# apchenstu/mvsnerf

Hardware: NVIDIA B200
Metric: rays/sec @ 128 samples, DTU 512x640 (higher is better)
Workload: dtype fp16 operands / fp32 accumulate

## Files before the change

### mvsnerf_b200/csrc/render_tc2.cu

```cuda
#include "render_frontend.cuh"
#include "umma.cuh"

namespace mvsn {

using namespace umma;

namespace tc2 {
constexpr int W_MOD = 0;
constexpr int W_L0 = 8192;
constexpr int W_L1 = 16384;
constexpr int L_STRIDE = 18432;
constexpr int W_L5 = W_L1 + 4 * L_STRIDE;
constexpr int W_V = W_L5 + 3 * 8192;
constexpr int W_V_TILE = 10240;
constexpr int W_RGB = W_V + 12288;
constexpr int HALF_BYTES = W_RGB + 1024;
constexpr int TAIL_OFFSET = 2 * HALF_BYTES;
constexpr int TOTAL_BYTES = TAIL_OFFSET + 16;
static_assert(W_L5 % 1024 == 0 && W_V % 1024 == 0 && W_RGB % 1024 == 0 && HALF_BYTES % 1024 == 0, "SW128 blocks need 1024-byte alignment");
constexpr int N_VIEWS_OP = 80;
}

namespace {

constexpr int THREADS = 544;
constexpr int OFF_SLOT = tc2::HALF_BYTES;
constexpr int SLOT_BYTES = 32768, OFF_PE = 0, OFF_MISC = 16384;
constexpr int OFF_XCH = OFF_SLOT + 2 * SLOT_BYTES;
constexpr int SMEM_BYTES = OFF_XCH + 2 * 2048 + 1024;
constexpr uint32_t COL_H = 128, COL_MOD = 192, COL_LZ = 128;

struct Shared {
    uint64_t in_ready[2];
    uint64_t pe_ready[2];
    uint64_t acc_ready[2];
    uint64_t pe_free[2];
    uint64_t misc_free[2];
    uint64_t w_full;
    uint32_t tmem_base;
    Cams cams;
};

__device__ __forceinline__ uint32_t pack_h2(float a, float b) {
    __half2 h = __floats2half2_rn(a, b);
    return *reinterpret_cast<uint32_t*>(&h);
}
__device__ __forceinline__ void named_bar_sync(int id, int nthreads) {
    asm volatile("bar.sync %0, %1;\n" ::"r"(id), "r"(nthreads) : "memory");
}
__device__ __forceinline__ void tmem_wait16(uint32_t (&r)[16]) {
    asm volatile("tcgen05.wait::ld.sync.aligned;\n"
                 : "+r"(r[0]), "+r"(r[1]), "+r"(r[2]), "+r"(r[3]), "+r"(r[4]), "+r"(r[5]), "+r"(r[6]), "+r"(r[7]),
                   "+r"(r[8]), "+r"(r[9]), "+r"(r[10]), "+r"(r[11]), "+r"(r[12]), "+r"(r[13]), "+r"(r[14]), "+r"(r[15])
                 :: "memory");
}
__device__ __forceinline__ void tmem_wait8(uint32_t (&r)[8]) {
    asm volatile("tcgen05.wait::ld.sync.aligned;\n"
                 : "+r"(r[0]), "+r"(r[1]), "+r"(r[2]), "+r"(r[3]), "+r"(r[4]), "+r"(r[5]), "+r"(r[6]), "+r"(r[7]) :: "memory");
}
__device__ __forceinline__ void tmem_ld8(uint32_t taddr, uint32_t (&r)[8]) {
    asm volatile("tcgen05.ld.sync.aligned.32x32b.x8.b32 {%0, %1, %2, %3, %4, %5, %6, %7}, [%8];\n"
                 : "=r"(r[0]), "=r"(r[1]), "=r"(r[2]), "=r"(r[3]), "=r"(r[4]), "=r"(r[5]), "=r"(r[6]), "=r"(r[7]) : "r"(taddr));
}
__device__ __forceinline__ void tmem_st8(uint32_t taddr, const uint32_t (&r)[8]) {
    asm volatile("tcgen05.st.sync.aligned.32x32b.x8.b32 [%0], {%1, %2, %3, %4, %5, %6, %7, %8};\n"
                 :: "r"(taddr), "r"(r[0]), "r"(r[1]), "r"(r[2]), "r"(r[3]), "r"(r[4]), "r"(r[5]), "r"(r[6]), "r"(r[7]) : "memory");
}

template <bool RELU>
__device__ __forceinline__ uint32_t cvt_h2(float lo, float hi) {
    uint32_t r;
    if (RELU) asm("cvt.rn.relu.satfinite.f16x2.f32 %0, %1, %2;\n" : "=r"(r) : "f"(hi), "f"(lo));
    else      asm("cvt.rn.satfinite.f16x2.f32 %0, %1, %2;\n" : "=r"(r) : "f"(hi), "f"(lo));
    return r;
}
__device__ __forceinline__ uint32_t mul_relu_h2(uint32_t a, uint32_t b) {
    uint32_t r;
    const uint32_t zero = 0u, maxh = 0x7BFF7BFFu;
    asm("fma.rn.relu.f16x2 %0, %1, %2, %3;\n" : "=r"(r) : "r"(a), "r"(b), "r"(zero));
    asm("min.f16x2 %0, %1, %2;\n" : "=r"(r) : "r"(r), "r"(maxh));
    return r;
}

__device__ __forceinline__ void epilogue_hidden(uint32_t t_acc, uint32_t t_mod, uint32_t t_h) {
    uint32_t a[2][16], m[2][8];
    tmem_ld16(t_acc, a[0]);
    tmem_ld8(t_mod, m[0]);
#pragma unroll
    for (int i = 0; i < 8; ++i) {
        tmem_wait16(a[i & 1]);
        tmem_wait8(m[i & 1]);
        if (i + 1 < 8) {
            tmem_ld16(t_acc + (i + 1) * 16, a[(i + 1) & 1]);
            tmem_ld8(t_mod + (i + 1) * 8, m[(i + 1) & 1]);
        }
        uint32_t o[8];
#pragma unroll
        for (int j = 0; j < 8; ++j)
            o[j] = mul_relu_h2(cvt_h2<false>(__uint_as_float(a[i & 1][2 * j]), __uint_as_float(a[i & 1][2 * j + 1])), m[i & 1][j]);
        tmem_st8(t_h + i * 8, o);
    }
}

#ifdef MVSN_TC_TRACE
#define TC_TRACE(ev) do { if (tr && tr_n < 1023) tr[tr_n++] = (clock64() << 8) | (long long)(ev); } while (0)
#else
#define TC_TRACE(ev) do { } while (0)
#endif

template <bool FAST>
__global__ void __cluster_dims__(2, 1, 1) __launch_bounds__(THREADS, 1)
render_tc2_kernel(const SceneDev sc, const RenderIO io, const uint8_t* __restrict__ wimg) {
    extern __shared__ uint8_t smem_raw[];
    uint8_t* smem = smem_raw + ((1024u - (smem_u32(smem_raw) & 1023u)) & 1023u);
    __shared__ Shared sh;
    const int tid = threadIdx.x, warp = tid >> 5, lane = tid & 31;
    const uint32_t rank = cluster_ctarank();

    load_cams(sc, &sh.cams, tid);
    if (tid == 0) {
        for (int s = 0; s < 2; ++s) {
            mbar_init(&sh.in_ready[s], 8);
            mbar_init(&sh.pe_ready[s], 8);
            mbar_init(&sh.acc_ready[s], 1);
            mbar_init(&sh.pe_free[s], 1);
            mbar_init(&sh.misc_free[s], 1);
        }
        mbar_init(&sh.w_full, 1);
        fence_barrier_init();
    }
    if (warp == 16) { tmem_alloc_pair(&sh.tmem_base, 512); tmem_relinquish_pair(); }
    __syncthreads();
    if (tid == 0) {
        mbar_arrive_expect_tx(&sh.w_full, (uint32_t)tc2::HALF_BYTES);
        const uint8_t* src = wimg + (size_t)rank * tc2::HALF_BYTES;
        for (int i = 0; i < 4; ++i) bulk_load(smem + i * 32000, src + i * 32000, 32000u, &sh.w_full);
    }
    mbar_wait(&sh.w_full, 0);
    tc_fence_before();
    __syncthreads();
    cluster_sync_all();
    tc_fence_after();
    const uint32_t tmem = sh.tmem_base;
#ifdef MVSN_TC_TRACE
    long long* tr = nullptr; int tr_n = 0;
    if (io.trace && blockIdx.x == 0 && lane == 0) {
        if (warp < 16 && (warp & 3) == 0) tr = io.trace + (warp >> 2) * 1024;
        else if (warp == 16) tr = io.trace + 4 * 1024;
    }
#endif

    const int N = io.N, S = io.S;
    const int RT = io.rays_per_tile, SP = 128 / RT;
    const int rt_shift = 31 - __clz(RT);
    const int NT = (S + SP - 1) / SP;
    const int G = (N + RT - 1) / RT;
    const int npairs = (int)gridDim.x >> 1, pair = (int)blockIdx.x >> 1;
    const int n_gpass = (G + npairs * 4 - 1) / (npairs * 4);
    auto group_of = [&](int gp, int s, int r) { return ((gp * npairs + pair) * 2 + s) * 2 + r; };
    auto slot_active = [&](int gp, int s) { return group_of(gp, s, 0) < G; };

    if (warp < 8) {
        const int s = warp >> 2, wq = warp & 3, row = wq * 32 + lane;
        const uint32_t t_acc = tmem + ((uint32_t)(wq * 32) << 16) + (uint32_t)(s * 256);
        const uint32_t t_h = t_acc + COL_H, t_mod = t_acc + COL_MOD, t_lz = t_acc + COL_LZ;
        const uint32_t leader_in_ready = mapa_u32(smem_u32(&sh.in_ready[s]), 0);
        uint32_t par_acc = 0;
        float cT = 1.f, c0 = 0.f, c1 = 0.f, c2 = 0.f, c3 = 0.f, c4 = 0.f;
        const float br0 = __ldg(reinterpret_cast<const float*>(wimg + tc2::TAIL_OFFSET));
        const float br1 = __ldg(reinterpret_cast<const float*>(wimg + tc2::TAIL_OFFSET) + 1);
        const float br2 = __ldg(reinterpret_cast<const float*>(wimg + tc2::TAIL_OFFSET) + 2);
        float4* xch = reinterpret_cast<float4*>(smem + OFF_XCH + s * 2048);

        auto signal = [&]() {
            tc_fence_before();
            __syncwarp();
            if (lane == 0) mbar_arrive_cluster(leader_in_ready);
        };
        signal();

#pragma unroll 1
        for (int gp = 0; gp < n_gpass; ++gp) {
            if (!slot_active(gp, s)) continue;
            const int g = group_of(gp, s, (int)rank);
#pragma unroll 1
            for (int tile = 0; tile < NT; ++tile) {
                mbar_wait(&sh.acc_ready[s], par_acc); par_acc ^= 1;
                TC_TRACE(10);
                tc_fence_after();
                {
                    uint32_t mu[32], t[2][16];
                    tmem_ld16(t_lz + 64, t[0]);
#pragma unroll
                    for (int i = 0; i < 4; ++i) {
                        tmem_wait16(t[i & 1]);
                        tmem_ld16(i + 1 < 4 ? t_lz + 64 + (i + 1) * 16 : t_lz, t[(i + 1) & 1]);
#pragma unroll
                        for (int j = 0; j < 8; ++j)
                            mu[i * 8 + j] = cvt_h2<false>(__uint_as_float(t[i & 1][2 * j]), __uint_as_float(t[i & 1][2 * j + 1]));
                    }
#pragma unroll
                    for (int i = 0; i < 4; ++i) {
                        tmem_wait16(t[i & 1]);
                        if (i + 1 < 4) tmem_ld16(t_lz + (i + 1) * 16, t[(i + 1) & 1]);
                        uint32_t o[8];
#pragma unroll
                        for (int j = 0; j < 8; ++j)
                            o[j] = cvt_h2<false>(__uint_as_float(t[i & 1][2 * j]), __uint_as_float(t[i & 1][2 * j + 1]));
                        tmem_st8(t_mod + i * 8, o);
                    }
#pragma unroll
                    for (int i = 0; i < 4; ++i) {
                        uint32_t o[8];
#pragma unroll
                        for (int j = 0; j < 8; ++j) o[j] = mu[i * 8 + j];
                        tmem_st8(t_mod + 32 + i * 8, o);
                    }
                    tmem_st_wait();
                }
                epilogue_hidden(t_acc, t_mod, t_h);
                tmem_st_wait();
                TC_TRACE(30);
                signal();
#pragma unroll 1
                for (int op = 1; op < 6; ++op) {
                    mbar_wait(&sh.acc_ready[s], par_acc); par_acc ^= 1;
                    TC_TRACE(10 + op);
                    tc_fence_after();
                    epilogue_hidden(t_acc, t_mod, t_h);
                    tmem_st_wait();
                    TC_TRACE(30 + op);
                    signal();
                }
                float sigma;
                {
                    mbar_wait(&sh.acc_ready[s], par_acc); par_acc ^= 1;
                    TC_TRACE(16);
                    tc_fence_after();
                    uint32_t a[2][16];
                    tmem_ld16(t_acc, a[0]);
#pragma unroll
                    for (int i = 0; i < 4; ++i) {
                        tmem_wait16(a[i & 1]);
                        tmem_ld16(t_acc + (i + 1) * 16, a[(i + 1) & 1]);
                        uint32_t o[8];
#pragma unroll
                        for (int j = 0; j < 8; ++j)
                            o[j] = cvt_h2<true>(__uint_as_float(a[i & 1][2 * j]), __uint_as_float(a[i & 1][2 * j + 1]));
                        tmem_st8(t_h + i * 8, o);
                    }
                    tmem_wait16(a[0]);
                    sigma = fmaxf(__uint_as_float(a[0][0]), 0.f);
                    tmem_st_wait();
                    TC_TRACE(36);
                    signal();
                }
                float cr, cg, cb;
                {
                    mbar_wait(&sh.acc_ready[s], par_acc); par_acc ^= 1;
                    TC_TRACE(17);
                    tc_fence_after();
                    uint32_t r16[16];
                    tmem_ld16(t_acc, r16);
                    tmem_wait16(r16);
                    signal();
                    cr = __fdividef(1.f, 1.f + __expf(-(__uint_as_float(r16[0]) + br0)));
                    cg = __fdividef(1.f, 1.f + __expf(-(__uint_as_float(r16[1]) + br1)));
                    cb = __fdividef(1.f, 1.f + __expf(-(__uint_as_float(r16[2]) + br2)));
                }
                xch[row] = make_float4(1.f - __expf(-sigma), cr, cg, cb);
                named_bar_sync(1 + s, 128);
                if (row < RT) {
                    if (tile == 0) { cT = 1.f; c0 = c1 = c2 = c3 = c4 = 0.f; }
                    const int cray = g * RT + row;
                    if (cray < N) {
                        float znear = 0.f, zfar = 0.f;
                        if (FAST) { const float4 r1 = __ldg(reinterpret_cast<const float4*>(io.rays + (size_t)cray * 8) + 1); znear = r1.z; zfar = r1.w; }
                        for (int sub = 0; sub < SP; ++sub) {
                            const int sj = tile * SP + sub;
                            if (sj >= S) break;
                            const float4 v = xch[sub * RT + row];
                            float z;
                            if (FAST) {
                                const float t = __ldg(io.t_steps + sj);
                                if (!io.rg.lindisp) z = __fadd_rn(__fmul_rn(znear, 1.f - t), __fmul_rn(zfar, t));
                                else z = __fdiv_rn(1.f, __fadd_rn(__fmul_rn(__fdiv_rn(1.f, znear), 1.f - t), __fmul_rn(__fdiv_rn(1.f, zfar), t)));
                            } else {
                                z = __ldg(io.z + (size_t)cray * S + sj);
                            }
                            const float wgt = v.x * cT;
                            if (io.alpha) io.alpha[(size_t)cray * S + sj] = v.x;
                            if (io.weights) io.weights[(size_t)cray * S + sj] = wgt;
                            c0 = fmaf(wgt, v.y, c0); c1 = fmaf(wgt, v.z, c1); c2 = fmaf(wgt, v.w, c2);
                            c3 = fmaf(wgt, z, c3); c4 += wgt;
                            cT *= (1.f - v.x) + 1e-10f;
                        }
                        if (tile == NT - 1) {
                            float o0 = c0, o1 = c1, o2 = c2;
                            if (sc.white_bkgd) { const float bg = 1.f - c4; o0 += bg; o1 += bg; o2 += bg; }
                            store_pixel(io, cray, o0, o1, o2, c3);
                        }
                    }
                }
                TC_TRACE(53);
            }
        }
    } else if (warp < 16) {
        const int s = (warp - 8) >> 2, row = ((warp - 8) & 3) * 32 + lane;
        uint8_t* slot = smem + OFF_SLOT + s * SLOT_BYTES;
        const uint32_t leader_pe_ready = mapa_u32(smem_u32(&sh.pe_ready[s]), 0);
        uint32_t tcount = 0;
#pragma unroll 1
        for (int gp = 0; gp < n_gpass; ++gp) {
            if (!slot_active(gp, s)) continue;
            const int g = group_of(gp, s, (int)rank);
#pragma unroll 1
            for (int tile = 0; tile < NT; ++tile, ++tcount) {
                TC_TRACE(1);
                const int r_in = row & (RT - 1), s_idx = tile * SP + (row >> rt_shift);
                const int ray = g * RT + r_in;
                const bool valid = g < G && ray < N && s_idx < S;
                const size_t si = (size_t)ray * S + s_idx;
                float nx = 0.f, ny = 0.f, nz = 0.f;
                float px = 0.f, py = 0.f, pz = 0.f, dx = 0.f, dy = 0.f, dz = 1.f;
                if (valid) {
                    if (FAST) {
                        const float4* rp = reinterpret_cast<const float4*>(io.rays + (size_t)ray * 8);
                        const float4 r0 = __ldg(rp), r1 = __ldg(rp + 1);
                        dx = r0.w; dy = r1.x; dz = r1.y;
                        const float near = r1.z, far = r1.w, t = __ldg(io.t_steps + s_idx);
                        float zv;
                        if (!io.rg.lindisp) zv = __fadd_rn(__fmul_rn(near, 1.f - t), __fmul_rn(far, t));
                        else zv = __fdiv_rn(1.f, __fadd_rn(__fmul_rn(__fdiv_rn(1.f, near), 1.f - t),
                                                           __fmul_rn(__fdiv_rn(1.f, far), t)));
                        px = __fadd_rn(r0.x, __fmul_rn(dx, zv));
                        py = __fadd_rn(r0.y, __fmul_rn(dy, zv));
                        pz = __fadd_rn(r0.z, __fmul_rn(dz, zv));
                        ndc_of_point<false>(sc, sh.cams, io.rg, px, py, pz, nx, ny, nz);
                    } else {
                        px = __ldg(io.pts + si * 3); py = __ldg(io.pts + si * 3 + 1); pz = __ldg(io.pts + si * 3 + 2);
                        nx = __ldg(io.ndc + si * 3); ny = __ldg(io.ndc + si * 3 + 1); nz = __ldg(io.ndc + si * 3 + 2);
                        dx = __ldg(io.dirs + (size_t)ray * 3); dy = __ldg(io.dirs + (size_t)ray * 3 + 1);
                        dz = __ldg(io.dirs + (size_t)ray * 3 + 2);
                    }
                }
                uint4 mc[3];
                uint32_t md0, md1;
                {
                    float feat[20], dir[3] = {0.f, 0.f, 0.f};
#pragma unroll
                    for (int i = 0; i < 20; ++i) feat[i] = 0.f;
                    if (valid) {
                        view_dir<false>(sh.cams, dx, dy, dz, dir);
                        sample_volume_2pass(sc, nx, ny, nz, feat);
#pragma unroll
// ... 9 lines not shown
                    mc[1] = make_uint4(pack_h2(feat[8], feat[9]), pack_h2(feat[10], feat[11]), pack_h2(feat[12], feat[13]), pack_h2(feat[14], feat[15]));
                    mc[2] = make_uint4(pack_h2(feat[16], feat[17]), pack_h2(feat[18], feat[19]), pack_h2(1.f, 0.f), 0u);
                    md0 = pack_h2(dir[0], dir[1]); md1 = pack_h2(dir[2], 1.f);
                }
                TC_TRACE(4);
                uint4 pc[8];
                {
                    const float nd[3] = {nx, ny, nz};
                    auto pe = [&](int i) -> float {
                        if (i < 3) return nd[i];
                        if (i < 33) return __sinf(nd[(i - 3) % 3] * (float)(1 << ((i - 3) / 3)));
                        if (i < 63) return __cosf(nd[(i - 33) % 3] * (float)(1 << ((i - 33) / 3)));
                        return 1.f;
                    };
#pragma unroll
                    for (int c = 0; c < 8; ++c)
                        pc[c] = make_uint4(pack_h2(pe(c * 8), pe(c * 8 + 1)), pack_h2(pe(c * 8 + 2), pe(c * 8 + 3)),
                                           pack_h2(pe(c * 8 + 4), pe(c * 8 + 5)), pack_h2(pe(c * 8 + 6), pe(c * 8 + 7)));
                }
                TC_TRACE(5);
                if (tcount > 0) mbar_wait(&sh.pe_free[s], (tcount - 1) & 1);
#pragma unroll
                for (int c = 0; c < 8; ++c) *reinterpret_cast<uint4*>(slot + OFF_PE + sw128_offset(row, c * 8)) = pc[c];
                if (tcount > 0) mbar_wait(&sh.misc_free[s], (tcount - 1) & 1);
                uint8_t* m = slot + OFF_MISC;
                *reinterpret_cast<uint4*>(m + sw128_offset(row, 0)) = mc[0];
                *reinterpret_cast<uint4*>(m + sw128_offset(row, 8)) = mc[1];
                *reinterpret_cast<uint4*>(m + sw128_offset(row, 16)) = mc[2];
                *reinterpret_cast<uint4*>(m + sw128_offset(row, 24)) = make_uint4(0u, 0u, 0u, 0u);
                *reinterpret_cast<uint4*>(m + sw128_offset(row, 32)) = make_uint4(md0, md1, 0u, 0u);
                *reinterpret_cast<uint4*>(m + sw128_offset(row, 40)) = make_uint4(0u, 0u, 0u, 0u);
                fence_proxy_async();
                __syncwarp();
                if (lane == 0) mbar_arrive_cluster(leader_pe_ready);
                TC_TRACE(2);
            }
        }
    } else if (rank == 0) {
        const bool leader = elect_one();
        const uint32_t sbase = smem_u32(smem);
        constexpr uint32_t HI_SW = (uint32_t)(desc_sw128(0) >> 32), HI_NS = (uint32_t)(desc_nosw(0, 128, 256) >> 32);
        constexpr uint32_t LO_SW = (uint32_t)desc_sw128(0), LO_NS = (uint32_t)desc_nosw(0, 128, 256);
        auto dsw = [&](uint32_t addr) { return ((uint64_t)HI_SW << 32) | (uint64_t)(LO_SW | (addr >> 4)); };
        auto dns = [&](uint32_t addr) { return ((uint64_t)HI_NS << 32) | (uint64_t)(LO_NS | (addr >> 4)); };
        constexpr uint32_t ID128 = idesc_f16(256, 128), IDV = idesc_f16(256, tc2::N_VIEWS_OP), IDR = idesc_f16(256, 16);
        uint32_t par_in[2] = {0, 0}, par_pe[2] = {0, 0};
#pragma unroll 1
        for (int gp = 0; gp < n_gpass; ++gp) {
            const bool act[2] = {slot_active(gp, 0), slot_active(gp, 1)};
#pragma unroll 1
            for (int tile = 0; tile < NT; ++tile) {
#pragma unroll 1
                for (int op = 0; op < 8; ++op) {
#pragma unroll
                    for (int s = 0; s < 2; ++s) {
                        if (!act[s]) continue;
                        if (op == 0) { mbar_wait_cluster(&sh.pe_ready[s], par_pe[s]); par_pe[s] ^= 1; }
                        TC_TRACE(100 + op * 2 + s);
                        mbar_wait_cluster(&sh.in_ready[s], par_in[s]); par_in[s] ^= 1;
                        TC_TRACE(140 + op * 2 + s);
                        tc_fence_after();
                        if (leader) {
                            const uint32_t d_acc = tmem + (uint32_t)(s * 256);
                            const uint32_t a_h = d_acc + COL_H;
                            const uint32_t pe = sbase + OFF_SLOT + s * SLOT_BYTES + OFF_PE, misc = pe + OFF_MISC;
                            if (op == 0) {
                                const uint64_t dm = dsw(misc), dwm = dsw(sbase + tc2::W_MOD);
                                mma_f16_pair(d_acc + COL_LZ, dm, dwm, ID128, 0u);
                                mma_f16_pair(d_acc + COL_LZ, dm + 2, dwm + 2, ID128, 1u);
                                const uint64_t dp = dsw(pe), dw0 = dsw(sbase + tc2::W_L0);
#pragma unroll
                                for (int ks = 0; ks < 4; ++ks) mma_f16_pair(d_acc, dp + 2 * ks, dw0 + 2 * ks, ID128, ks ? 1u : 0u);
                            } else if (op <= 4) {
                                const uint32_t wl = sbase + tc2::W_L1 + (op - 1) * tc2::L_STRIDE;
#pragma unroll
                                for (int kb = 0; kb < 2; ++kb) {
                                    const uint64_t dw = dsw(wl + kb * 8192);
#pragma unroll
                                    for (int ks = 0; ks < 4; ++ks)
                                        mma_f16_ts_pair(d_acc, a_h + (uint32_t)((kb * 4 + ks) * 8), dw + 2 * ks, ID128, (kb | ks) ? 1u : 0u);
                                }
                                mma_f16_pair(d_acc, dsw(misc) + 2, dns(wl + 16384), ID128, 1u);
                            } else if (op == 5) {
                                const uint64_t dp = dsw(pe), dw5 = dsw(sbase + tc2::W_L5);
#pragma unroll
                                for (int ks = 0; ks < 4; ++ks) mma_f16_pair(d_acc, dp + 2 * ks, dw5 + 2 * ks, ID128, ks ? 1u : 0u);
#pragma unroll
                                for (int kb = 0; kb < 2; ++kb) {
                                    const uint64_t dw = dsw(sbase + tc2::W_L5 + 8192 + kb * 8192);
#pragma unroll
                                    for (int ks = 0; ks < 4; ++ks)
                                        mma_f16_ts_pair(d_acc, a_h + (uint32_t)((kb * 4 + ks) * 8), dw + 2 * ks, ID128, 1u);
                                }
                            } else if (op == 6) {
#pragma unroll
                                for (int kb = 0; kb < 2; ++kb) {
                                    const uint64_t dw = dsw(sbase + tc2::W_V + kb * 5120);
#pragma unroll
                                    for (int ks = 0; ks < 4; ++ks)
                                        mma_f16_ts_pair(d_acc, a_h + (uint32_t)((kb * 4 + ks) * 8), dw + 2 * ks, IDV, (kb | ks) ? 1u : 0u);
                                }
                                mma_f16_pair(d_acc, dsw(misc) + 4, dns(sbase + tc2::W_V + tc2::W_V_TILE), IDV, 1u);
                            } else {
                                const uint64_t dw = dsw(sbase + tc2::W_RGB);
#pragma unroll
                                for (int ks = 0; ks < 4; ++ks) mma_f16_ts_pair(d_acc, a_h + (uint32_t)(ks * 8), dw + 2 * ks, IDR, ks ? 1u : 0u);
                            }
                            TC_TRACE(80 + op * 2 + s);
                            mma_commit_pair(&sh.acc_ready[s]);
                            if (op == 5) mma_commit_pair(&sh.pe_free[s]);
                            if (op == 6) mma_commit_pair(&sh.misc_free[s]);
                        }
                        __syncwarp();
                    }
                }
                TC_TRACE(200);
            }
        }
    }
    tc_fence_before();
    __syncthreads();
    cluster_sync_all();
    if (warp == 16) tmem_dealloc_pair(tmem, 512);
}

}

int launch_render_tc2(const SceneDev& sc, const RenderIO& io_in, bool fast, const void* wimg, cudaStream_t stream) {
    RenderIO io = io_in;
    static bool attr_set[64] = {false};
    int dev = 0;
    MVSN_CUDA_CHECK(cudaGetDevice(&dev));
    if (dev >= 64 || !attr_set[dev]) {
        MVSN_CUDA_CHECK(cudaFuncSetAttribute(render_tc2_kernel<true>, cudaFuncAttributeMaxDynamicSharedMemorySize, SMEM_BYTES));
        MVSN_CUDA_CHECK(cudaFuncSetAttribute(render_tc2_kernel<false>, cudaFuncAttributeMaxDynamicSharedMemorySize, SMEM_BYTES));
        if (dev < 64) attr_set[dev] = true;
    }
    const int max_pairs = sm_count() / 2;
    int rt = 32;
    while (rt > 4 && (io.N + rt - 1) / rt < 4 * max_pairs) rt >>= 1;
    io.rays_per_tile = rt;
    const int G = (io.N + rt - 1) / rt;
    int pairs = (G + 3) / 4;
    if (pairs > max_pairs) pairs = max_pairs;
    if (pairs <= 0) return MVSN_OK;
    const uint8_t* w = static_cast<const uint8_t*>(wimg);
    if (fast) render_tc2_kernel<true><<<2 * pairs, THREADS, SMEM_BYTES, stream>>>(sc, io, w);
    else      render_tc2_kernel<false><<<2 * pairs, THREADS, SMEM_BYTES, stream>>>(sc, io, w);
    MVSN_CUDA_CHECK(cudaGetLastError());
    return MVSN_OK;
}

struct MlpPtrsTc2 { const float* p[MVSN_N_MLP_TENSORS]; };

__device__ __forceinline__ uint32_t nosw_offset2(int r, int k) {
    return (uint32_t)((r >> 3) * 256 + (k >> 3) * 128 + (r & 7) * 16 + (k & 7) * 2);
}

__global__ void pack_mlp_tc2_kernel(MlpPtrsTc2 w, uint8_t* __restrict__ out) {
    const int rank = blockIdx.x / 9, reg = blockIdx.x % 9;
    const int tid = threadIdx.x, nt = blockDim.x;
    int off, bytes;
    if (reg == 0) { off = tc2::W_MOD; bytes = 8192; }
    else if (reg == 1) { off = tc2::W_L0; bytes = 8192; }
    else if (reg <= 5) { off = tc2::W_L1 + (reg - 2) * tc2::L_STRIDE; bytes = tc2::L_STRIDE; }
    else if (reg == 6) { off = tc2::W_L5; bytes = 3 * 8192; }
    else if (reg == 7) { off = tc2::W_V; bytes = 12288; }
    else { off = tc2::W_RGB; bytes = 1024; }
    uint8_t* dst = out + (size_t)rank * tc2::HALF_BYTES + off;
    for (int i = tid * 16; i < bytes; i += nt * 16) *reinterpret_cast<uint4*>(dst + i) = make_uint4(0, 0, 0, 0);
    __syncthreads();
    auto put = [&](uint32_t o, float v) { *reinterpret_cast<__half*>(dst + o) = __float2half_rn(v); };
    if (reg == 0) {
        for (int i = tid; i < 64 * 21; i += nt) { const int lr = i / 21, k = i % 21, n = rank * 64 + lr;
            put(sw128_offset(lr, k), k < 20 ? w.p[12][n * 20 + k] : w.p[13][n]); }
    } else if (reg == 1) {
        for (int i = tid; i < 64 * 64; i += nt) { const int lr = i / 64, k = i % 64, n = rank * 64 + lr;
            put(sw128_offset(lr, k), k < 63 ? w.p[0][n * 63 + k] : w.p[1][n]); }
    } else if (reg <= 5) {
        const int l = reg - 1;
        for (int i = tid; i < 64 * 128; i += nt) { const int lr = i / 128, k = i % 128, n = rank * 64 + lr;
            put((k >> 6) * 8192 + sw128_offset(lr, k & 63), w.p[2 * l][n * 128 + k]); }
        for (int lr = tid; lr < 64; lr += nt) put(16384 + nosw_offset2(lr, 4), w.p[2 * l + 1][rank * 64 + lr]);
    } else if (reg == 6) {
        for (int i = tid; i < 64 * 64; i += nt) { const int lr = i / 64, k = i % 64, n = rank * 64 + lr;
            put(sw128_offset(lr, k), k < 63 ? w.p[10][n * 191 + k] : w.p[11][n]); }
        for (int i = tid; i < 64 * 128; i += nt) { const int lr = i / 128, k = i % 128, n = rank * 64 + lr;
            put(8192 + (k >> 6) * 8192 + sw128_offset(lr, k & 63), w.p[10][n * 191 + 63 + k]); }
    } else if (reg == 7) {
        for (int i = tid; i < 40 * 128; i += nt) {
            const int lr = i / 128, k = i % 128, n = rank * 40 + lr;
            float v = 0.f;
            if (n < 64) {
                double acc = 0.0;
                for (int j = 0; j < 128; ++j) acc += (double)w.p[14][n * 131 + j] * (double)w.p[16][j * 128 + k];
                v = (float)acc;
            } else if (n == 64) {
                v = w.p[18][k];
            }
            put((k >> 6) * 5120 + sw128_offset(lr, k & 63), v);
        }
        for (int i = tid; i < 40 * 4; i += nt) {
            const int lr = i / 4, k = i % 4, n = rank * 40 + lr;
            float v = 0.f;
            if (n < 64) {
                if (k < 3) v = w.p[14][n * 131 + 128 + k];
                else {
                    double acc = (double)w.p[15][n];
// ... 27 lines not shown
```

### mvsnerf_b200/csrc/umma.cuh

```cuda
#pragma once
#include <cuda_fp16.h>
#include <cstdint>

namespace mvsn {
namespace umma {

__device__ __forceinline__ uint32_t smem_u32(const void* p) { return (uint32_t)__cvta_generic_to_shared(p); }

__device__ __forceinline__ bool elect_one() {
    uint32_t pred;
    asm volatile(
        "{\n\t"
        ".reg .pred P;\n\t"
        "elect.sync _|P, 0xffffffff;\n\t"
        "selp.b32 %0, 1, 0, P;\n\t"
        "}\n" : "=r"(pred));
    return pred != 0;
}

__device__ __forceinline__ void mbar_init(uint64_t* bar, uint32_t count) {
    asm volatile("mbarrier.init.shared::cta.b64 [%0], %1;\n" ::"r"(smem_u32(bar)), "r"(count) : "memory");
}
__device__ __forceinline__ void fence_barrier_init() { asm volatile("fence.mbarrier_init.release.cluster;\n" ::: "memory"); }
__device__ __forceinline__ void mbar_arrive(uint64_t* bar) {
// ... 32 lines not shown
    asm volatile(
        "{\n\t"
        ".reg .pred P1;\n\t"
        "mbarrier.try_wait.parity.acquire.cluster.shared::cta.b64 P1, [%1], %2, 0xF4240;\n\t"
        "selp.b32 %0, 1, 0, P1;\n\t"
        "}\n" : "=r"(ok) : "r"(addr), "r"(parity) : "memory");
    return ok != 0;
}
__device__ __forceinline__ void mbar_wait_cluster(uint64_t* bar, uint32_t parity) {
    const uint32_t addr = smem_u32(bar);
    if (mbar_try_wait_cluster(addr, parity)) return;
    const uint64_t t0 = global_timer_ns();
    while (!mbar_try_wait_cluster(addr, parity))
        if (global_timer_ns() - t0 > MVSN_MBAR_TIMEOUT_NS) __trap();
}

__device__ __forceinline__ uint32_t cluster_ctarank() {
    uint32_t r;
    asm volatile("mov.u32 %0, %%cluster_ctarank;\n" : "=r"(r));
    return r;
}
__device__ __forceinline__ void cluster_sync_all() {
    asm volatile("barrier.cluster.arrive.release.aligned;\n" ::: "memory");
    asm volatile("barrier.cluster.wait.acquire.aligned;\n" ::: "memory");
}
__device__ __forceinline__ uint32_t mapa_u32(uint32_t local_smem_addr, uint32_t rank) {
    uint32_t r;
    asm volatile("mapa.shared::cluster.u32 %0, %1, %2;\n" : "=r"(r) : "r"(local_smem_addr), "r"(rank));
    return r;
}
__device__ __forceinline__ void mbar_arrive_cluster(uint32_t cluster_addr) {
    asm volatile("mbarrier.arrive.release.cluster.shared::cluster.b64 _, [%0];\n" ::"r"(cluster_addr) : "memory");
}

__device__ __forceinline__ void fence_proxy_async() { asm volatile("fence.proxy.async.shared::cta;\n" ::: "memory"); }
__device__ __forceinline__ void tc_fence_before() { asm volatile("tcgen05.fence::before_thread_sync;\n" ::: "memory"); }
__device__ __forceinline__ void tc_fence_after() { asm volatile("tcgen05.fence::after_thread_sync;\n" ::: "memory"); }

__device__ __forceinline__ void bulk_load(void* smem_dst, const void* gsrc, uint32_t bytes, uint64_t* bar) {
    asm volatile("cp.async.bulk.shared::cluster.global.mbarrier::complete_tx::bytes [%0], [%1], %2, [%3];\n"
                 ::"r"(smem_u32(smem_dst)), "l"(gsrc), "r"(bytes), "r"(smem_u32(bar)) : "memory");
}

__device__ __forceinline__ void tmem_alloc(uint32_t* holder, uint32_t ncols) {
    asm volatile("tcgen05.alloc.cta_group::1.sync.aligned.shared::cta.b32 [%0], %1;\n" ::"r"(smem_u32(holder)), "r"(ncols) : "memory");
}
__device__ __forceinline__ void tmem_relinquish() { asm volatile("tcgen05.relinquish_alloc_permit.cta_group::1.sync.aligned;\n" ::: "memory"); }
__device__ __forceinline__ void tmem_dealloc(uint32_t addr, uint32_t ncols) {
    asm volatile("tcgen05.dealloc.cta_group::1.sync.aligned.b32 %0, %1;\n" ::"r"(addr), "r"(ncols) : "memory");
}

__host__ __device__ constexpr uint64_t desc_sw128(uint32_t saddr) {
    uint64_t d = 0;
    d |= (uint64_t)((saddr >> 4) & 0x3FFF);
    d |= (uint64_t)1 << 16;
    d |= (uint64_t)(1024 >> 4) << 32;
    d |= (uint64_t)1 << 46;
    d |= (uint64_t)2 << 61;
    return d;
}
__host__ __device__ constexpr uint64_t desc_nosw(uint32_t saddr, uint32_t lbo, uint32_t sbo) {
    uint64_t d = 0;
    d |= (uint64_t)((saddr >> 4) & 0x3FFF);
    d |= (uint64_t)((lbo >> 4) & 0x3FFF) << 16;
    d |= (uint64_t)((sbo >> 4) & 0x3FFF) << 32;
    d |= (uint64_t)1 << 46;
// ... 91 lines not shown
```

Baseline: 30.83 million.

## Move modulation MMA and fp16 repack off the epilogue critical path

The modulation GEMM now runs as its own pair of N=64 MMAs, issued ahead of time as soon as the producer warps signal misc data ready. Its fp32-to-fp16 conversion and TMEM repack move from the epilogue warps to the producer warps, gated by new mod_ready and misc_ready barriers. The depth values z are also precomputed per row before the accumulator wait and exchanged through shared memory, instead of each compositing thread recomputing them serially. This adds barriers, repacks the W_MOD weight layout into two halves, and uses a different TMEM column for LZ, which raises ordering and overlap risk.

Measured after the change: 30.82 million, median of 6. Within noise of the previous version (-0.0%).

```diff
diff --git a/mvsnerf_b200/csrc/render_tc2.cu b/mvsnerf_b200/csrc/render_tc2.cu
--- a/mvsnerf_b200/csrc/render_tc2.cu
+++ b/mvsnerf_b200/csrc/render_tc2.cu
@@ -7,6 +7,7 @@
 
 namespace tc2 {
 constexpr int W_MOD = 0;
+constexpr int W_MOD_HALF = 4096;
 constexpr int W_L0 = 8192;
 constexpr int W_L1 = 16384;
 constexpr int L_STRIDE = 18432;
@@ -27,11 +28,14 @@
 constexpr int OFF_SLOT = tc2::HALF_BYTES;
 constexpr int SLOT_BYTES = 32768, OFF_PE = 0, OFF_MISC = 16384;
 constexpr int OFF_XCH = OFF_SLOT + 2 * SLOT_BYTES;
-constexpr int SMEM_BYTES = OFF_XCH + 2 * 2048 + 1024;
-constexpr uint32_t COL_H = 128, COL_MOD = 192, COL_LZ = 128;
+constexpr int OFF_XZ = OFF_XCH + 2 * 2048;
+constexpr int SMEM_BYTES = OFF_XZ + 2 * 512 + 1024;
+constexpr uint32_t COL_H = 128, COL_MOD = 192, COL_LZ = 64;
 
 struct Shared {
     uint64_t in_ready[2];
+    uint64_t misc_ready[2];
+    uint64_t mod_ready[2];
     uint64_t pe_ready[2];
     uint64_t acc_ready[2];
     uint64_t pe_free[2];
@@ -121,6 +125,8 @@
     if (tid == 0) {
         for (int s = 0; s < 2; ++s) {
             mbar_init(&sh.in_ready[s], 8);
+            mbar_init(&sh.misc_ready[s], 8);
+            mbar_init(&sh.mod_ready[s], 1);
             mbar_init(&sh.pe_ready[s], 8);
             mbar_init(&sh.acc_ready[s], 1);
             mbar_init(&sh.pe_free[s], 1);
@@ -147,6 +153,7 @@
     if (io.trace && blockIdx.x == 0 && lane == 0) {
         if (warp < 16 && (warp & 3) == 0) tr = io.trace + (warp >> 2) * 1024;
         else if (warp == 16) tr = io.trace + 4 * 1024;
+        else if (warp < 4) tr = io.trace + (4 + warp) * 1024;
     }
 #endif
 
@@ -163,7 +170,7 @@
     if (warp < 8) {
         const int s = warp >> 2, wq = warp & 3, row = wq * 32 + lane;
         const uint32_t t_acc = tmem + ((uint32_t)(wq * 32) << 16) + (uint32_t)(s * 256);
-        const uint32_t t_h = t_acc + COL_H, t_mod = t_acc + COL_MOD, t_lz = t_acc + COL_LZ;
+        const uint32_t t_h = t_acc + COL_H, t_mod = t_acc + COL_MOD;
         const uint32_t leader_in_ready = mapa_u32(smem_u32(&sh.in_ready[s]), 0);
         uint32_t par_acc = 0;
         float cT = 1.f, c0 = 0.f, c1 = 0.f, c2 = 0.f, c3 = 0.f, c4 = 0.f;
@@ -171,6 +178,7 @@
         const float br1 = __ldg(reinterpret_cast<const float*>(wimg + tc2::TAIL_OFFSET) + 1);
         const float br2 = __ldg(reinterpret_cast<const float*>(wimg + tc2::TAIL_OFFSET) + 2);
         float4* xch = reinterpret_cast<float4*>(smem + OFF_XCH + s * 2048);
+        float* xz = reinterpret_cast<float*>(smem + OFF_XZ + s * 512);
 
         auto signal = [&]() {
             tc_fence_before();
@@ -185,43 +193,35 @@
             const int g = group_of(gp, s, (int)rank);
 #pragma unroll 1
             for (int tile = 0; tile < NT; ++tile) {
+                float2 nf = make_float2(0.f, 0.f);
+                float tz = 0.f;
+                bool zvalid;
+                {
+                    const int r_in = row & (RT - 1), s_idx = tile * SP + (row >> rt_shift);
+                    const int ray = g * RT + r_in;
+                    zvalid = ray < N && s_idx < S;
+                    if (zvalid) {
+                        if (FAST) {
+                            nf = __ldg(reinterpret_cast<const float2*>(io.rays + (size_t)ray * 8 + 6));
+                            tz = __ldg(io.t_steps + s_idx);
+                        } else {
+                            tz = __ldg(io.z + (size_t)ray * S + s_idx);
+                        }
+                    }
+                }
                 mbar_wait(&sh.acc_ready[s], par_acc); par_acc ^= 1;
                 TC_TRACE(10);
                 tc_fence_after();
-                {
-                    uint32_t mu[32], t[2][16];
-                    tmem_ld16(t_lz + 64, t[0]);
-#pragma unroll
-                    for (int i = 0; i < 4; ++i) {
-                        tmem_wait16(t[i & 1]);
-                        tmem_ld16(i + 1 < 4 ? t_lz + 64 + (i + 1) * 16 : t_lz, t[(i + 1) & 1]);
-#pragma unroll
-                        for (int j = 0; j < 8; ++j)
-                            mu[i * 8 + j] = cvt_h2<false>(__uint_as_float(t[i & 1][2 * j]), __uint_as_float(t[i & 1][2 * j + 1]));
-                    }
-#pragma unroll
-                    for (int i = 0; i < 4; ++i) {
-                        tmem_wait16(t[i & 1]);
-                        if (i + 1 < 4) tmem_ld16(t_lz + (i + 1) * 16, t[(i + 1) & 1]);
-                        uint32_t o[8];
-#pragma unroll
-                        for (int j = 0; j < 8; ++j)
-                            o[j] = cvt_h2<false>(__uint_as_float(t[i & 1][2 * j]), __uint_as_float(t[i & 1][2 * j + 1]));
-                        tmem_st8(t_mod + i * 8, o);
-                    }
-#pragma unroll
-                    for (int i = 0; i < 4; ++i) {
-                        uint32_t o[8];
-#pragma unroll
-                        for (int j = 0; j < 8; ++j) o[j] = mu[i * 8 + j];
-                        tmem_st8(t_mod + 32 + i * 8, o);
-                    }
-                    tmem_st_wait();
-                }
                 epilogue_hidden(t_acc, t_mod, t_h);
                 tmem_st_wait();
                 TC_TRACE(30);
                 signal();
+                float z = 0.f;
+                if (zvalid) {
+                    if (!FAST) z = tz;
+                    else if (!io.rg.lindisp) z = __fadd_rn(__fmul_rn(nf.x, 1.f - tz), __fmul_rn(nf.y, tz));
+                    else z = __fdiv_rn(1.f, __fadd_rn(__fmul_rn(__fdiv_rn(1.f, nf.x), 1.f - tz), __fmul_rn(__fdiv_rn(1.f, nf.y), tz)));
+                }
 #pragma unroll 1
                 for (int op = 1; op < 6; ++op) {
                     mbar_wait(&sh.acc_ready[s], par_acc); par_acc ^= 1;
@@ -263,38 +263,33 @@
                     uint32_t r16[16];
                     tmem_ld16(t_acc, r16);
                     tmem_wait16(r16);
+                    TC_TRACE(37);
                     signal();
                     cr = __fdividef(1.f, 1.f + __expf(-(__uint_as_float(r16[0]) + br0)));
                     cg = __fdividef(1.f, 1.f + __expf(-(__uint_as_float(r16[1]) + br1)));
                     cb = __fdividef(1.f, 1.f + __expf(-(__uint_as_float(r16[2]) + br2)));
                 }
                 xch[row] = make_float4(1.f - __expf(-sigma), cr, cg, cb);
+                xz[row] = z;
                 named_bar_sync(1 + s, 128);
+                TC_TRACE(50);
                 if (row < RT) {
                     if (tile == 0) { cT = 1.f; c0 = c1 = c2 = c3 = c4 = 0.f; }
                     const int cray = g * RT + row;
                     if (cray < N) {
-                        float znear = 0.f, zfar = 0.f;
-                        if (FAST) { const float4 r1 = __ldg(reinterpret_cast<const float4*>(io.rays + (size_t)cray * 8) + 1); znear = r1.z; zfar = r1.w; }
                         for (int sub = 0; sub < SP; ++sub) {
                             const int sj = tile * SP + sub;
                             if (sj >= S) break;
                             const float4 v = xch[sub * RT + row];
-                            float z;
-                            if (FAST) {
-                                const float t = __ldg(io.t_steps + sj);
-                                if (!io.rg.lindisp) z = __fadd_rn(__fmul_rn(znear, 1.f - t), __fmul_rn(zfar, t));
-                                else z = __fdiv_rn(1.f, __fadd_rn(__fmul_rn(__fdiv_rn(1.f, znear), 1.f - t), __fmul_rn(__fdiv_rn(1.f, zfar), t)));
-                            } else {
-                                z = __ldg(io.z + (size_t)cray * S + sj);
-                            }
+                            const float zs = xz[sub * RT + row];
                             const float wgt = v.x * cT;
                             if (io.alpha) io.alpha[(size_t)cray * S + sj] = v.x;
                             if (io.weights) io.weights[(size_t)cray * S + sj] = wgt;
                             c0 = fmaf(wgt, v.y, c0); c1 = fmaf(wgt, v.z, c1); c2 = fmaf(wgt, v.w, c2);
-                            c3 = fmaf(wgt, z, c3); c4 += wgt;
+                            c3 = fmaf(wgt, zs, c3); c4 += wgt;
                             cT *= (1.f - v.x) + 1e-10f;
                         }
+                        TC_TRACE(52);
                         if (tile == NT - 1) {
                             float o0 = c0, o1 = c1, o2 = c2;
                             if (sc.white_bkgd) { const float bg = 1.f - c4; o0 += bg; o1 += bg; o2 += bg; }
@@ -308,7 +303,9 @@
     } else if (warp < 16) {
         const int s = (warp - 8) >> 2, row = ((warp - 8) & 3) * 32 + lane;
         uint8_t* slot = smem + OFF_SLOT + s * SLOT_BYTES;
+        const uint32_t leader_misc_ready = mapa_u32(smem_u32(&sh.misc_ready[s]), 0);
         const uint32_t leader_pe_ready = mapa_u32(smem_u32(&sh.pe_ready[s]), 0);
+        const uint32_t t_slot = tmem + ((uint32_t)(((warp - 8) & 3) * 32) << 16) + (uint32_t)(s * 256);
         uint32_t tcount = 0;
 #pragma unroll 1
         for (int gp = 0; gp < n_gpass; ++gp) {
@@ -396,6 +393,43 @@
                 *reinterpret_cast<uint4*>(m + sw128_offset(row, 40)) = make_uint4(0u, 0u, 0u, 0u);
                 fence_proxy_async();
                 __syncwarp();
+                if (lane == 0) mbar_arrive_cluster(leader_misc_ready);
+                TC_TRACE(6);
+                mbar_wait(&sh.mod_ready[s], tcount & 1);
+                tc_fence_after();
+                {
+                    const uint32_t t_lo = t_slot + COL_LZ, t_hi = t_slot + COL_MOD;
+                    uint32_t mu[32], t[2][16];
+                    tmem_ld16(t_hi, t[0]);
+#pragma unroll
+                    for (int i = 0; i < 4; ++i) {
+                        tmem_wait16(t[i & 1]);
+                        tmem_ld16(i + 1 < 4 ? t_hi + (i + 1) * 16 : t_lo, t[(i + 1) & 1]);
+#pragma unroll
+                        for (int j = 0; j < 8; ++j)
+                            mu[i * 8 + j] = cvt_h2<false>(__uint_as_float(t[i & 1][2 * j]), __uint_as_float(t[i & 1][2 * j + 1]));
+                    }
+#pragma unroll
+                    for (int i = 0; i < 4; ++i) {
+                        tmem_wait16(t[i & 1]);
+                        if (i + 1 < 4) tmem_ld16(t_lo + (i + 1) * 16, t[(i + 1) & 1]);
+                        uint32_t o[8];
+#pragma unroll
+                        for (int j = 0; j < 8; ++j)
+                            o[j] = cvt_h2<false>(__uint_as_float(t[i & 1][2 * j]), __uint_as_float(t[i & 1][2 * j + 1]));
+                        tmem_st8(t_hi + i * 8, o);
+                    }
+#pragma unroll
+                    for (int i = 0; i < 4; ++i) {
+                        uint32_t o[8];
+#pragma unroll
+                        for (int j = 0; j < 8; ++j) o[j] = mu[i * 8 + j];
+                        tmem_st8(t_hi + 32 + i * 8, o);
+                    }
+                    tmem_st_wait();
+                }
+                tc_fence_before();
+                __syncwarp();
                 if (lane == 0) mbar_arrive_cluster(leader_pe_ready);
                 TC_TRACE(2);
             }
@@ -408,7 +442,26 @@
         auto dsw = [&](uint32_t addr) { return ((uint64_t)HI_SW << 32) | (uint64_t)(LO_SW | (addr >> 4)); };
         auto dns = [&](uint32_t addr) { return ((uint64_t)HI_NS << 32) | (uint64_t)(LO_NS | (addr >> 4)); };
         constexpr uint32_t ID128 = idesc_f16(256, 128), IDV = idesc_f16(256, tc2::N_VIEWS_OP), IDR = idesc_f16(256, 16);
-        uint32_t par_in[2] = {0, 0}, par_pe[2] = {0, 0};
+        constexpr uint32_t IDM = idesc_f16(256, 64);
+        uint32_t par_in[2] = {0, 0}, par_pe[2] = {0, 0}, par_misc[2] = {0, 0};
+        auto issue_mod = [&](int s) {
+            mbar_wait_cluster(&sh.misc_ready[s], par_misc[s]); par_misc[s] ^= 1;
+            tc_fence_after();
+            if (leader) {
+                const uint32_t d = tmem + (uint32_t)(s * 256);
+                const uint64_t dm = dsw(sbase + OFF_SLOT + s * SLOT_BYTES + OFF_MISC);
+#pragma unroll
+                for (int h = 0; h < 2; ++h) {
+                    const uint64_t dw = dsw(sbase + tc2::W_MOD + h * tc2::W_MOD_HALF);
+                    const uint32_t dh = d + (h ? COL_MOD : COL_LZ);
+                    mma_f16_pair(dh, dm, dw, IDM, 0u);
+                    mma_f16_pair(dh, dm + 2, dw + 2, IDM, 1u);
+                }
+                TC_TRACE(160 + s);
+                mma_commit_pair(&sh.mod_ready[s]);
+            }
+            __syncwarp();
+        };
 #pragma unroll 1
         for (int gp = 0; gp < n_gpass; ++gp) {
             const bool act[2] = {slot_active(gp, 0), slot_active(gp, 1)};
@@ -419,7 +472,10 @@
 #pragma unroll
                     for (int s = 0; s < 2; ++s) {
                         if (!act[s]) continue;
-                        if (op == 0) { mbar_wait_cluster(&sh.pe_ready[s], par_pe[s]); par_pe[s] ^= 1; }
+                        if (op == 0) {
+                            if (gp == 0 && tile == 0) issue_mod(s);
+                            mbar_wait_cluster(&sh.pe_ready[s], par_pe[s]); par_pe[s] ^= 1;
+                        }
                         TC_TRACE(100 + op * 2 + s);
                         mbar_wait_cluster(&sh.in_ready[s], par_in[s]); par_in[s] ^= 1;
                         TC_TRACE(140 + op * 2 + s);
@@ -429,9 +485,6 @@
                             const uint32_t a_h = d_acc + COL_H;
                             const uint32_t pe = sbase + OFF_SLOT + s * SLOT_BYTES + OFF_PE, misc = pe + OFF_MISC;
                             if (op == 0) {
-                                const uint64_t dm = dsw(misc), dwm = dsw(sbase + tc2::W_MOD);
-                                mma_f16_pair(d_acc + COL_LZ, dm, dwm, ID128, 0u);
-                                mma_f16_pair(d_acc + COL_LZ, dm + 2, dwm + 2, ID128, 1u);
                                 const uint64_t dp = dsw(pe), dw0 = dsw(sbase + tc2::W_L0);
 #pragma unroll
                                 for (int ks = 0; ks < 4; ++ks) mma_f16_pair(d_acc, dp + 2 * ks, dw0 + 2 * ks, ID128, ks ? 1u : 0u);
@@ -476,6 +529,7 @@
                             if (op == 6) mma_commit_pair(&sh.misc_free[s]);
                         }
                         __syncwarp();
+                        if (op == 7 && (tile + 1 < NT || slot_active(gp + 1, s))) issue_mod(s);
                     }
                 }
                 TC_TRACE(200);
@@ -536,8 +590,8 @@
     __syncthreads();
     auto put = [&](uint32_t o, float v) { *reinterpret_cast<__half*>(dst + o) = __float2half_rn(v); };
     if (reg == 0) {
-        for (int i = tid; i < 64 * 21; i += nt) { const int lr = i / 21, k = i % 21, n = rank * 64 + lr;
-            put(sw128_offset(lr, k), k < 20 ? w.p[12][n * 20 + k] : w.p[13][n]); }
+        for (int i = tid; i < 64 * 21; i += nt) { const int lr = i / 21, k = i % 21, h = lr >> 5, n = h * 64 + rank * 32 + (lr & 31);
+            put(h * tc2::W_MOD_HALF + sw128_offset(lr & 31, k), k < 20 ? w.p[12][n * 20 + k] : w.p[13][n]); }
     } else if (reg == 1) {
         for (int i = tid; i < 64 * 64; i += nt) { const int lr = i / 64, k = i % 64, n = rank * 64 + lr;
             put(sw128_offset(lr, k), k < 63 ? w.p[0][n * 63 + k] : w.p[1][n]); }
```

## Rebalance registers between warp roles and widen the TMEM epilogue loads

Applied to the files above, without the earlier changes.

Epilogue warps now raise their register limit with setmaxnreg.inc, and producer warps lower theirs with setmaxnreg.dec. Per-block work indices move into a Work struct built inside each role, and the bias loads are deferred to the RGB step. These changes are meant to cut register pressure and spills in the epilogue. The hidden-layer epilogue now uses 32-column TMEM loads and 16-column stores in 4 iterations instead of 8, so there are fewer load/wait round trips at the cost of more live registers. The risk is spilling, or producer warps being starved at 72 registers. The setmaxnreg budget also has to match what the compiler allocates, and the MMA warp never adjusts its own count.

Measured after the change: 30.95 million before, 29.80 million after, median of 6. 3.7% lower.

```diff
diff --git a/mvsnerf_b200/csrc/render_tc2.cu b/mvsnerf_b200/csrc/render_tc2.cu
--- a/mvsnerf_b200/csrc/render_tc2.cu
+++ b/mvsnerf_b200/csrc/render_tc2.cu
@@ -30,6 +30,9 @@
 constexpr int SMEM_BYTES = OFF_XCH + 2 * 2048 + 1024;
 constexpr uint32_t COL_H = 128, COL_MOD = 192, COL_LZ = 128;
 
+constexpr uint32_t REG_EPI = 120, REG_PROD = 72;
+static_assert(8 * REG_EPI + 8 * REG_PROD + 96 <= 17 * 96 && REG_EPI % 8 == 0 && REG_PROD % 8 == 0, "register budget");
+
 struct Shared {
     uint64_t in_ready[2];
     uint64_t pe_ready[2];
@@ -54,6 +57,14 @@
                    "+r"(r[8]), "+r"(r[9]), "+r"(r[10]), "+r"(r[11]), "+r"(r[12]), "+r"(r[13]), "+r"(r[14]), "+r"(r[15])
                  :: "memory");
 }
+__device__ __forceinline__ void tmem_wait32(uint32_t (&r)[32]) {
+    asm volatile("tcgen05.wait::ld.sync.aligned;\n"
+                 : "+r"(r[0]), "+r"(r[1]), "+r"(r[2]), "+r"(r[3]), "+r"(r[4]), "+r"(r[5]), "+r"(r[6]), "+r"(r[7]),
+                   "+r"(r[8]), "+r"(r[9]), "+r"(r[10]), "+r"(r[11]), "+r"(r[12]), "+r"(r[13]), "+r"(r[14]), "+r"(r[15]),
+                   "+r"(r[16]), "+r"(r[17]), "+r"(r[18]), "+r"(r[19]), "+r"(r[20]), "+r"(r[21]), "+r"(r[22]), "+r"(r[23]),
+                   "+r"(r[24]), "+r"(r[25]), "+r"(r[26]), "+r"(r[27]), "+r"(r[28]), "+r"(r[29]), "+r"(r[30]), "+r"(r[31])
+                 :: "memory");
+}
 __device__ __forceinline__ void tmem_wait8(uint32_t (&r)[8]) {
     asm volatile("tcgen05.wait::ld.sync.aligned;\n"
                  : "+r"(r[0]), "+r"(r[1]), "+r"(r[2]), "+r"(r[3]), "+r"(r[4]), "+r"(r[5]), "+r"(r[6]), "+r"(r[7]) :: "memory");
@@ -82,6 +93,30 @@
     return r;
 }
 
+#ifndef EPI_CW
+#define EPI_CW 32
+#endif
+#if EPI_CW == 32
+__device__ __forceinline__ void epilogue_hidden(uint32_t t_acc, uint32_t t_mod, uint32_t t_h) {
+    uint32_t a[2][32], m[2][16];
+    tmem_ld32(t_acc, a[0]);
+    tmem_ld16(t_mod, m[0]);
+#pragma unroll
+    for (int i = 0; i < 4; ++i) {
+        tmem_wait32(a[i & 1]);
+        tmem_wait16(m[i & 1]);
+        if (i + 1 < 4) {
+            tmem_ld32(t_acc + (i + 1) * 32, a[(i + 1) & 1]);
+            tmem_ld16(t_mod + (i + 1) * 16, m[(i + 1) & 1]);
+        }
+        uint32_t o[16];
+#pragma unroll
+        for (int j = 0; j < 16; ++j)
+            o[j] = mul_relu_h2(cvt_h2<false>(__uint_as_float(a[i & 1][2 * j]), __uint_as_float(a[i & 1][2 * j + 1])), m[i & 1][j]);
+        tmem_st16(t_h + i * 16, o);
+    }
+}
+#else
 __device__ __forceinline__ void epilogue_hidden(uint32_t t_acc, uint32_t t_mod, uint32_t t_h) {
     uint32_t a[2][16], m[2][8];
     tmem_ld16(t_acc, a[0]);
@@ -101,12 +136,28 @@
         tmem_st8(t_h + i * 8, o);
     }
 }
+#endif
 
 #ifdef MVSN_TC_TRACE
 #define TC_TRACE(ev) do { if (tr && tr_n < 1023) tr[tr_n++] = (clock64() << 8) | (long long)(ev); } while (0)
 #else
 #define TC_TRACE(ev) do { } while (0)
 #endif
+
+struct Work {
+    int N, S, RT, SP, rt_shift, NT, G, npairs, pair, n_gpass;
+    __device__ __forceinline__ Work(int n, int s, int rt) : N(n), S(s), RT(rt) {
+        SP = 128 / RT;
+        rt_shift = 31 - __clz(RT);
+        NT = (S + SP - 1) / SP;
+        G = (N + RT - 1) / RT;
+        npairs = (int)gridDim.x >> 1;
+        pair = (int)blockIdx.x >> 1;
+        n_gpass = (G + npairs * 4 - 1) / (npairs * 4);
+    }
+    __device__ __forceinline__ int group_of(int gp, int s, int r) const { return ((gp * npairs + pair) * 2 + s) * 2 + r; }
+    __device__ __forceinline__ bool slot_active(int gp, int s) const { return group_of(gp, s, 0) < G; }
+};
 
 template <bool FAST>
 __global__ void __cluster_dims__(2, 1, 1) __launch_bounds__(THREADS, 1)
@@ -150,26 +201,15 @@
     }
 #endif
 
-    const int N = io.N, S = io.S;
-    const int RT = io.rays_per_tile, SP = 128 / RT;
-    const int rt_shift = 31 - __clz(RT);
-    const int NT = (S + SP - 1) / SP;
-    const int G = (N + RT - 1) / RT;
-    const int npairs = (int)gridDim.x >> 1, pair = (int)blockIdx.x >> 1;
-    const int n_gpass = (G + npairs * 4 - 1) / (npairs * 4);
-    auto group_of = [&](int gp, int s, int r) { return ((gp * npairs + pair) * 2 + s) * 2 + r; };
-    auto slot_active = [&](int gp, int s) { return group_of(gp, s, 0) < G; };
-
     if (warp < 8) {
+        setmaxnreg_inc<REG_EPI>();
+        const Work wk(io.N, io.S, io.rays_per_tile);
         const int s = warp >> 2, wq = warp & 3, row = wq * 32 + lane;
         const uint32_t t_acc = tmem + ((uint32_t)(wq * 32) << 16) + (uint32_t)(s * 256);
         const uint32_t t_h = t_acc + COL_H, t_mod = t_acc + COL_MOD, t_lz = t_acc + COL_LZ;
         const uint32_t leader_in_ready = mapa_u32(smem_u32(&sh.in_ready[s]), 0);
         uint32_t par_acc = 0;
         float cT = 1.f, c0 = 0.f, c1 = 0.f, c2 = 0.f, c3 = 0.f, c4 = 0.f;
-        const float br0 = __ldg(reinterpret_cast<const float*>(wimg + tc2::TAIL_OFFSET));
-        const float br1 = __ldg(reinterpret_cast<const float*>(wimg + tc2::TAIL_OFFSET) + 1);
-        const float br2 = __ldg(reinterpret_cast<const float*>(wimg + tc2::TAIL_OFFSET) + 2);
         float4* xch = reinterpret_cast<float4*>(smem + OFF_XCH + s * 2048);
 
         auto signal = [&]() {
@@ -180,11 +220,11 @@
         signal();
 
 #pragma unroll 1
-        for (int gp = 0; gp < n_gpass; ++gp) {
-            if (!slot_active(gp, s)) continue;
-            const int g = group_of(gp, s, (int)rank);
-#pragma unroll 1
-            for (int tile = 0; tile < NT; ++tile) {
+        for (int gp = 0; gp < wk.n_gpass; ++gp) {
+            if (!wk.slot_active(gp, s)) continue;
+            const int g = wk.group_of(gp, s, (int)rank);
+#pragma unroll 1
+            for (int tile = 0; tile < wk.NT; ++tile) {
                 mbar_wait(&sh.acc_ready[s], par_acc); par_acc ^= 1;
                 TC_TRACE(10);
                 tc_fence_after();
@@ -264,38 +304,40 @@
                     tmem_ld16(t_acc, r16);
                     tmem_wait16(r16);
                     signal();
+                    const float* br = reinterpret_cast<const float*>(wimg + tc2::TAIL_OFFSET);
+                    const float br0 = __ldg(br), br1 = __ldg(br + 1), br2 = __ldg(br + 2);
                     cr = __fdividef(1.f, 1.f + __expf(-(__uint_as_float(r16[0]) + br0)));
                     cg = __fdividef(1.f, 1.f + __expf(-(__uint_as_float(r16[1]) + br1)));
                     cb = __fdividef(1.f, 1.f + __expf(-(__uint_as_float(r16[2]) + br2)));
                 }
                 xch[row] = make_float4(1.f - __expf(-sigma), cr, cg, cb);
                 named_bar_sync(1 + s, 128);
-                if (row < RT) {
+                if (row < wk.RT) {
                     if (tile == 0) { cT = 1.f; c0 = c1 = c2 = c3 = c4 = 0.f; }
-                    const int cray = g * RT + row;
-                    if (cray < N) {
+                    const int cray = g * wk.RT + row;
+                    if (cray < wk.N) {
                         float znear = 0.f, zfar = 0.f;
                         if (FAST) { const float4 r1 = __ldg(reinterpret_cast<const float4*>(io.rays + (size_t)cray * 8) + 1); znear = r1.z; zfar = r1.w; }
-                        for (int sub = 0; sub < SP; ++sub) {
-                            const int sj = tile * SP + sub;
-                            if (sj >= S) break;
-                            const float4 v = xch[sub * RT + row];
+                        for (int sub = 0; sub < wk.SP; ++sub) {
+                            const int sj = tile * wk.SP + sub;
+                            if (sj >= wk.S) break;
+                            const float4 v = xch[sub * wk.RT + row];
                             float z;
                             if (FAST) {
                                 const float t = __ldg(io.t_steps + sj);
                                 if (!io.rg.lindisp) z = __fadd_rn(__fmul_rn(znear, 1.f - t), __fmul_rn(zfar, t));
                                 else z = __fdiv_rn(1.f, __fadd_rn(__fmul_rn(__fdiv_rn(1.f, znear), 1.f - t), __fmul_rn(__fdiv_rn(1.f, zfar), t)));
                             } else {
-                                z = __ldg(io.z + (size_t)cray * S + sj);
+                                z = __ldg(io.z + (size_t)cray * wk.S + sj);
                             }
                             const float wgt = v.x * cT;
-                            if (io.alpha) io.alpha[(size_t)cray * S + sj] = v.x;
-                            if (io.weights) io.weights[(size_t)cray * S + sj] = wgt;
+                            if (io.alpha) io.alpha[(size_t)cray * wk.S + sj] = v.x;
+                            if (io.weights) io.weights[(size_t)cray * wk.S + sj] = wgt;
                             c0 = fmaf(wgt, v.y, c0); c1 = fmaf(wgt, v.z, c1); c2 = fmaf(wgt, v.w, c2);
                             c3 = fmaf(wgt, z, c3); c4 += wgt;
                             cT *= (1.f - v.x) + 1e-10f;
                         }
-                        if (tile == NT - 1) {
+                        if (tile == wk.NT - 1) {
                             float o0 = c0, o1 = c1, o2 = c2;
                             if (sc.white_bkgd) { const float bg = 1.f - c4; o0 += bg; o1 += bg; o2 += bg; }
                             store_pixel(io, cray, o0, o1, o2, c3);
@@ -306,21 +348,23 @@
             }
         }
     } else if (warp < 16) {
+        setmaxnreg_dec<REG_PROD>();
+        const Work wk(io.N, io.S, io.rays_per_tile);
         const int s = (warp - 8) >> 2, row = ((warp - 8) & 3) * 32 + lane;
         uint8_t* slot = smem + OFF_SLOT + s * SLOT_BYTES;
         const uint32_t leader_pe_ready = mapa_u32(smem_u32(&sh.pe_ready[s]), 0);
         uint32_t tcount = 0;
 #pragma unroll 1
-        for (int gp = 0; gp < n_gpass; ++gp) {
-            if (!slot_active(gp, s)) continue;
-            const int g = group_of(gp, s, (int)rank);
-#pragma unroll 1
-            for (int tile = 0; tile < NT; ++tile, ++tcount) {
+        for (int gp = 0; gp < wk.n_gpass; ++gp) {
+            if (!wk.slot_active(gp, s)) continue;
+            const int g = wk.group_of(gp, s, (int)rank);
+#pragma unroll 1
+            for (int tile = 0; tile < wk.NT; ++tile, ++tcount) {
                 TC_TRACE(1);
-                const int r_in = row & (RT - 1), s_idx = tile * SP + (row >> rt_shift);
-                const int ray = g * RT + r_in;
-                const bool valid = g < G && ray < N && s_idx < S;
-                const size_t si = (size_t)ray * S + s_idx;
+                const int r_in = row & (wk.RT - 1), s_idx = tile * wk.SP + (row >> wk.rt_shift);
+                const int ray = g * wk.RT + r_in;
+                const bool valid = g < wk.G && ray < wk.N && s_idx < wk.S;
+                const size_t si = (size_t)ray * wk.S + s_idx;
                 float nx = 0.f, ny = 0.f, nz = 0.f;
                 float px = 0.f, py = 0.f, pz = 0.f, dx = 0.f, dy = 0.f, dz = 1.f;
                 if (valid) {
@@ -401,6 +445,7 @@
             }
         }
     } else if (rank == 0) {
+        const Work wk(io.N, io.S, io.rays_per_tile);
         const bool leader = elect_one();
         const uint32_t sbase = smem_u32(smem);
         constexpr uint32_t HI_SW = (uint32_t)(desc_sw128(0) >> 32), HI_NS = (uint32_t)(desc_nosw(0, 128, 256) >> 32);
@@ -410,10 +455,10 @@
         constexpr uint32_t ID128 = idesc_f16(256, 128), IDV = idesc_f16(256, tc2::N_VIEWS_OP), IDR = idesc_f16(256, 16);
         uint32_t par_in[2] = {0, 0}, par_pe[2] = {0, 0};
 #pragma unroll 1
-        for (int gp = 0; gp < n_gpass; ++gp) {
-            const bool act[2] = {slot_active(gp, 0), slot_active(gp, 1)};
-#pragma unroll 1
-            for (int tile = 0; tile < NT; ++tile) {
+        for (int gp = 0; gp < wk.n_gpass; ++gp) {
+            const bool act[2] = {wk.slot_active(gp, 0), wk.slot_active(gp, 1)};
+#pragma unroll 1
+            for (int tile = 0; tile < wk.NT; ++tile) {
 #pragma unroll 1
                 for (int op = 0; op < 8; ++op) {
 #pragma unroll
diff --git a/mvsnerf_b200/csrc/umma.cuh b/mvsnerf_b200/csrc/umma.cuh
--- a/mvsnerf_b200/csrc/umma.cuh
+++ b/mvsnerf_b200/csrc/umma.cuh
@@ -88,6 +88,9 @@
 __device__ __forceinline__ void mbar_arrive_cluster(uint32_t cluster_addr) {
     asm volatile("mbarrier.arrive.release.cluster.shared::cluster.b64 _, [%0];\n" ::"r"(cluster_addr) : "memory");
 }
+
+template <uint32_t N> __device__ __forceinline__ void setmaxnreg_inc() { asm volatile("setmaxnreg.inc.sync.aligned.u32 %0;\n" ::"n"(N)); }
+template <uint32_t N> __device__ __forceinline__ void setmaxnreg_dec() { asm volatile("setmaxnreg.dec.sync.aligned.u32 %0;\n" ::"n"(N)); }
 
 __device__ __forceinline__ void fence_proxy_async() { asm volatile("fence.proxy.async.shared::cta;\n" ::: "memory"); }
 __device__ __forceinline__ void tc_fence_before() { asm volatile("tcgen05.fence::before_thread_sync;\n" ::: "memory"); }
```
